# klausondrag/FOSVOS

Measured on AMD Instinct MI355X. Metric: online fine-tune frames/sec (854x480), higher is better.
Workload: dtype bf16; 1 GPU; OSVOS_VGG train_online one-shot fine-tune: 1x3x480x854 frame per step, fwd + class-balanced BCE + bwd, fused SGD step every 5 steps (BASELINE.json configs[1]); batch=1, avg_grad_every_n=5, activations=bf16 NHWC, fp32 accumulate, fp32 master weights, parallelism=single GPU

## Files before the change

fosvos_amd/csrc/common.hpp:

```cpp
#pragma once
#include <hip/hip_runtime.h>
#include <stdarg.h>
#include <algorithm>
#include <stdint.h>
#include <stdio.h>
#include <stdlib.h>
#include <string.h>

#include "../../include/fosvos_hip.h"

namespace fosvos {

extern thread_local char g_err[512];

inline int fail(int code, const char *fmt, ...) __attribute__((format(printf, 2, 3)));
inline int fail(int code, const char *fmt, ...) {
    va_list ap;
    va_start(ap, fmt);
    vsnprintf(g_err, sizeof(g_err), fmt, ap);
    va_end(ap);
    return code;
}

#define FOSVOS_HIP_CHECK(expr)                                                                         \
// ... 19 lines not shown
    } while (0)
#define FOSVOS_LAUNCH_CHECK()                            \
    do {                                                 \
        if (::fosvos::g_prof_on) ::fosvos::prof_end();   \
        FOSVOS_HIP_CHECK(hipGetLastError());             \
    } while (0)

struct WgradReduceEntry {
    const float *slabs;
    float *dw, *db;
    const float *bias_part;
    int64_t E_real, E_pad;
    int S, S_bias, Co, Cor, accumulate;
    int block_begin, n_blocks;
    int fold_begin, fold_blocks;
};
constexpr int kWgradReduceMax = 20;
struct WgradReduceTable {
    int n;
    WgradReduceEntry e[kWgradReduceMax];
};
int wgrad_impl(const uint16_t *x, const uint16_t *dy, float *dw, float *db, int N, int H, int W, int Ci, int Co,
               int accumulate, void *workspace, size_t workspace_bytes, int device, void *stream,
               WgradReduceTable *reduce, bool alone = false);
int first_wgrad_impl(const float *frame, const uint16_t *dy, float *dw, float *db, int N, int H, int W, int Co,
                     int accumulate, void *workspace, size_t workspace_bytes, int device, void *stream,
                     WgradReduceTable *reduce);
int wgrad_reduce_all(WgradReduceTable *reduce, int device, void *stream);
int wgrad_queue_reduce(const float *slabs, const float *bias_part, float *dw, float *db, int S, int S_bias, int64_t E_real,
                       int64_t E_pad, int Co, int Cor, int accumulate, WgradReduceTable *reduce, int device, void *stream);
struct HeadBwdArgs {
    const float *const *side;
    const int *hs, *ws;
    const float *const *filt, *const *filt1;
    const float *dsn_w, *fuse_w, *d_fused;
    const float *const *d_side_out;
    uint16_t *const *d_side;
    float *d_fuse_w, *d_fuse_b, *d_dsn_w, *d_dsn_b;
    int N, H, W, accumulate;
    void *workspace;
    size_t workspace_bytes;
    int device;
    int filt_uniform;
};
int head_bwd_check(const HeadBwdArgs &a);
int head_bwd_scale(const HeadBwdArgs &a, int s, void *stream);
int head_bwd_finish(const HeadBwdArgs &a, void *stream);
// ... 179 lines not shown
```

fosvos_amd/csrc/conv_wgrad.hip:

```cpp
#include <stdlib.h>

#include "common.hpp"

using namespace fosvos;

namespace {
constexpr int TH = 8;
constexpr int TPIX = TH * 16;
constexpr int HALO_W = 18;
constexpr int BCI = 64;

struct WgArgs {
    const uint16_t *x;
    const uint16_t *dy;
    float *slabs;
    float *bias_part;
    int N, H, W, Ci, Cy, Cor;
    int tiles_x, tiles_y, n_tiles, tiles_per_split;
    int lab;
    int S, n_ci, n_co, xcd_order;
};

typedef __attribute__((address_space(3))) s16x4 *lds_s16x4_ptr;

// ... 16 lines not shown
    static constexpr int NXIT = (X_PIECES + NW - 1) / NW;
    static constexpr int N_IT = 2 + NXIT;
    static_assert(Y_PIECES == 2 * NW, "two dy pieces per wave, four tile rows apart");
};

typedef __attribute__((address_space(3))) void lds_void;

__device__ __forceinline__ bf16x8 tr_pair16(const char *p, int second) {
    const s16x4 lo = __builtin_amdgcn_ds_read_tr16_b64_v4i16((lds_s16x4_ptr)(p));
    const s16x4 hi = __builtin_amdgcn_ds_read_tr16_b64_v4i16((lds_s16x4_ptr)(p + second));
    typedef __attribute__((ext_vector_type(8))) short s16x8;
    const s16x8 v = __builtin_shufflevector(lo, hi, 0, 1, 2, 3, 4, 5, 6, 7);
    return __builtin_bit_cast(bf16x8, v);
}

#pragma clang diagnostic push
#pragma clang diagnostic ignored "-Winline-asm"
__device__ __forceinline__ void dma16(const __amdgpu_buffer_rsrc_t rsrc, unsigned lds_dst, unsigned voff, unsigned soff) {
    asm volatile("s_mov_b32 m0, %0\n\ts_nop 0\n\tbuffer_load_dwordx4 %1, %2, %3 offen lds"
                 :: "s"(lds_dst), "v"(voff), "s"(rsrc), "s"(soff) : "memory", "m0");
}
#pragma clang diagnostic pop

template <bool SIDE>
__global__ __launch_bounds__(Cfg2<SIDE>::NT) __attribute__((amdgpu_waves_per_eu(SIDE ? 2 : 3, SIDE ? 4 : 3))) void k_wgrad3x3_v2(const WgArgs a) {
    using C = Cfg2<SIDE>;
    constexpr int NW = C::NW, NU = C::NU, YPX = C::YPX, Y_BYTES = C::Y_BYTES, BUF_BYTES = C::BUF_BYTES, N_IT = C::N_IT;
    extern __shared__ __attribute__((aligned(16))) char smem_w[];
    const int tid = threadIdx.x, lane = tid & 63;
    const int wave = __builtin_amdgcn_readfirstlane(tid >> 6);
    const int wc = SIDE ? 0 : wave >> 2, wi = wave & 3;
    int bid = blockIdx.x;
    if (a.xcd_order) {
        const int n_wg = gridDim.x, q8 = n_wg >> 3, r8 = n_wg & 7, xcd = bid & 7;
        bid = (xcd < r8 ? xcd * (q8 + 1) : r8 * (q8 + 1) + (xcd - r8) * q8) + (bid >> 3);
    }
    const int co_blk = bid % a.n_co, ci_blk = (bid / a.n_co) % a.n_ci, split = bid / (a.n_co * a.n_ci);
    const int ci0 = ci_blk * 64, co0 = co_blk * C::BCO;
    const int H = a.H, W = a.W;
    const unsigned lds0 = __builtin_amdgcn_readfirstlane((unsigned)(size_t)(lds_void *)smem_w);

    f32x4 acc[9][NU];
#pragma unroll
    for (int t = 0; t < 9; ++t)
#pragma unroll
        for (int u = 0; u < NU; ++u) acc[t][u] = f32x4{0.f, 0.f, 0.f, 0.f};
    float bsum[NU];
#pragma unroll
    for (int u = 0; u < NU; ++u) bsum[u] = 0.f;

    const int g = lane >> 4, q = (lane & 15) >> 2, p = lane & 3;
    const int pxl = 4 * (g & 1) + q;
    auto swz128 = [](int px, int c) { return (c ^ (2 * ((px >> 1) & 3))) * 16; };
    auto swz64 = [](int px, int c) { return (c ^ (2 * ((px >> 2) & 1))) * 16; };
    int rd_y[NU], rd_x[3];
#pragma unroll
    for (int u = 0; u < NU; ++u)
        rd_y[u] = ((4 * (g >> 1)) * 16 + pxl) * YPX + (SIDE ? swz64(pxl, p >> 1) : swz128(pxl, 2 * (2 * wc + u) + (p >> 1))) + (p & 1) * 8;
#pragma unroll
    for (int kx = 0; kx < 3; ++kx)
        rd_x[kx] = Y_BYTES + ((4 * (g >> 1)) * XROW + pxl + kx) * 128 + swz128(pxl + kx, 2 * wi + (p >> 1)) + (p & 1) * 8;
// ... 53 lines not shown
        if (++lt_y == a.tiles_y) { lt_y = 0; ++lt_n; }                                                          \
    }
#define FOSVOS_W2_PIECE_ANY(it_, img_)                                                                          \
    if constexpr ((it_) < 2) { FOSVOS_W2_PIECE_Y(it_, img_) }                                                   \
    else if constexpr ((it_) < N_IT) { FOSVOS_W2_PIECE_X(it_, img_) }
#define FOSVOS_W2_STAGE(img_)                                                                                   \
    {                                                                                                           \
        FOSVOS_W2_TILE_SCALARS()                                                                                \
        FOSVOS_W2_PIECE_ANY(0, img_) FOSVOS_W2_PIECE_ANY(1, img_) FOSVOS_W2_PIECE_ANY(2, img_)                  \
        FOSVOS_W2_PIECE_ANY(3, img_) FOSVOS_W2_PIECE_ANY(4, img_) FOSVOS_W2_PIECE_ANY(5, img_)                  \
        FOSVOS_W2_PIECE_ANY(6, img_) FOSVOS_W2_PIECE_ANY(7, img_) FOSVOS_W2_PIECE_ANY(8, img_)                  \
        FOSVOS_W2_PIECE_ANY(9, img_)                                                                            \
        FOSVOS_W2_ADVANCE()                                                                                     \
    }
    static_assert(N_IT <= 10, "piece macros cover ten pieces per wave");
#define FOSVOS_W2_PIECES_OF_ROW(R, img_)                                                                        \
    if (has_next) { FOSVOS_W2_PIECE_ANY(2 * (R), img_) FOSVOS_W2_PIECE_ANY(2 * (R) + 1, img_) }

    if (t_begin < t_end) FOSVOS_W2_STAGE(lds0)
    asm volatile("s_waitcnt vmcnt(0)" ::: "memory");
    __syncthreads();

    const bool do_bias = a.bias_part != nullptr;
    typedef __attribute__((ext_vector_type(2))) __bf16 bf16x2_t;
    auto add8 = [](const bf16x8 &f, float acc_) {
        const bf16x2_t one2 = __builtin_bit_cast(bf16x2_t, 0x3f803f80u);
        acc_ = __builtin_amdgcn_fdot2_f32_bf16(__builtin_shufflevector(f, f, 0, 1), one2, acc_, false);
        acc_ = __builtin_amdgcn_fdot2_f32_bf16(__builtin_shufflevector(f, f, 2, 3), one2, acc_, false);
        acc_ = __builtin_amdgcn_fdot2_f32_bf16(__builtin_shufflevector(f, f, 4, 5), one2, acc_, false);
        acc_ = __builtin_amdgcn_fdot2_f32_bf16(__builtin_shufflevector(f, f, 6, 7), one2, acc_, false);
        return acc_;
    };

    for (int tile = t_begin; tile < t_end; ++tile) {
        const int par = (tile - t_begin) & 1;
        const char *cur = smem_w + par * BUF_BYTES;
        const bool has_next = tile + 1 < t_end;
        const unsigned nxt_ = lds0 + (par ^ 1) * BUF_BYTES;
        FOSVOS_W2_TILE_SCALARS()
        const bool my_bias = do_bias && (tile % a.n_ci) == ci_blk && ((tile / a.n_ci) & 3) == wi;

        const char *yb[NU];
#pragma unroll
        for (int u = 0; u < NU; ++u) yb[u] = cur + rd_y[u];
        const char *xb0 = cur + rd_x[0], *xb1 = cur + rd_x[1], *xb2 = cur + rd_x[2];
        bf16x8 a0[NU], a1[NU], a2[NU], b[3], bn[3];
#pragma unroll
        for (int u = 0; u < NU; ++u) a0[u] = a1[u] = a2[u] = bf16x8{};
        bn[0] = bn[1] = bn[2] = bf16x8{};
        b[0] = tr_pair16(xb0, 1024);
        b[1] = tr_pair16(xb1, 1024);
        b[2] = tr_pair16(xb2, 1024);
#define FOSVOS_W2_ROW(R)                                                                                        \
        {                                                                                                           \
            _Pragma("unroll") for (int u = 0; u < NU; ++u) { a2[u] = a1[u]; a1[u] = a0[u]; }                        \
// ... 14 lines not shown
            }                                                                                                       \
            if constexpr ((R) >= 1 && (R) <= 4) {                                                                   \
                _Pragma("unroll") for (int kx = 0; kx < 3; ++kx)                                                    \
                _Pragma("unroll") for (int u = 0; u < NU; ++u)                                                      \
                    acc[3 + kx][u] = __builtin_amdgcn_mfma_f32_16x16x32_bf16(a1[u], b[kx], acc[3 + kx][u], 0, 0, 0); \
            }                                                                                                       \
            if constexpr ((R) < 4) {                                                                                \
                _Pragma("unroll") for (int kx = 0; kx < 3; ++kx)                                                    \
                _Pragma("unroll") for (int u = 0; u < NU; ++u)                                                      \
                    acc[kx][u] = __builtin_amdgcn_mfma_f32_16x16x32_bf16(a0[u], b[kx], acc[kx][u], 0, 0, 0);        \
                if (my_bias) {                                                                                      \
                    _Pragma("unroll") for (int u = 0; u < NU; ++u) bsum[u] = add8(a0[u], bsum[u]);                  \
                }                                                                                                   \
            }                                                                                                       \
            asm volatile("" ::: "memory");                                                                          \
            b[0] = bn[0]; b[1] = bn[1]; b[2] = bn[2];                                                               \
        }
        FOSVOS_W2_ROW(0) FOSVOS_W2_ROW(1) FOSVOS_W2_ROW(2) FOSVOS_W2_ROW(3) FOSVOS_W2_ROW(4) FOSVOS_W2_ROW(5)
        if (has_next) FOSVOS_W2_ADVANCE()
        asm volatile("s_waitcnt vmcnt(0)" ::: "memory");
        __syncthreads();
    }

    if (do_bias) {
        float *sb = reinterpret_cast<float *>(smem_w);
#pragma unroll
        for (int u = 0; u < NU; ++u) sb[(wi * 4 + g) * C::BCO + wc * 32 + u * 16 + (lane & 15)] = bsum[u];
        __syncthreads();
        if (tid < C::BCO && co0 + tid < a.Cor) {
            float acc_b = 0.f;
#pragma unroll
            for (int k = 0; k < 16; ++k) acc_b += sb[k * C::BCO + tid];
            a.bias_part[((int64_t)split * a.n_ci + ci_blk) * a.Cor + co0 + tid] = acc_b;
        }
    }
    float *slab = a.slabs + (int64_t)split * a.Cor * a.Ci * 9;
    const int ci = ci0 + wi * 16 + (lane & 15);
#pragma unroll
    for (int u = 0; u < NU; ++u)
#pragma unroll
        for (int r = 0; r < 4; ++r) {
            const int co = co0 + wc * 32 + u * 16 + 4 * g + r;
            if (co >= a.Cor || (a.lab & 1)) continue;
            float *d = slab + ((int64_t)co * a.Ci + ci) * 9;
#pragma unroll
            for (int t = 0; t < 9; ++t) d[t] = acc[t][u][r];
        }
#undef FOSVOS_W2_ROW
#undef FOSVOS_W2_PIECES_OF_ROW
#undef FOSVOS_W2_PIECE_ANY
#undef FOSVOS_W2_TILE_SCALARS
#undef FOSVOS_W2_ADVANCE
#undef FOSVOS_W2_STAGE
#undef FOSVOS_W2_PIECE_X
#undef FOSVOS_W2_PIECE_Y
}
}

constexpr int kFold = 8;

__global__ __launch_bounds__(256) void k_wgrad_fold(const WgradReduceTable t) {
    int e = 0;
    while (e + 1 < t.n && (int)blockIdx.x >= t.e[e + 1].fold_begin) ++e;
    const WgradReduceEntry &q = t.e[e];
    const int local = blockIdx.x - q.fold_begin;
    if (local >= q.fold_blocks) return;
    const int per_group = q.n_blocks;
    const int grp = local / per_group;
    const int64_t i4 = (int64_t)(local - grp * per_group) * 256 + threadIdx.x;
    if (i4 * 4 >= q.E_real) return;
    float *base = const_cast<float *>(q.slabs) + (int64_t)grp * kFold * q.E_pad + i4 * 4;
    const int n = min(kFold, q.S - grp * kFold);
    float4 v[kFold];
#pragma unroll
    for (int j = 0; j < kFold; ++j) v[j] = *reinterpret_cast<const float4 *>(base + (int64_t)min(j, n - 1) * q.E_pad);
    float4 acc = v[0];
#pragma unroll
    for (int j = 1; j < kFold; ++j)
// ... 73 lines not shown
    size_t slab_bytes, bias_bytes;
};

Plan make_plan(int N, int H, int W, int Ci, int Co, bool alone = false) {
    Plan p;
    p.side = Co % 64 != 0;
    p.Cor = p.side ? Co : roundup(Co, 64);
    p.Cy = roundup(Co, 32);
    p.tiles_x = (int)cdiv(W, 16);
    p.tiles_y = (int)cdiv(H, TH);
    p.n_tiles = p.tiles_x * p.tiles_y * N;
    const int out_blocks = p.side ? Ci / 64 : (p.Cor / 64) * (Ci / 64);
    int S = (int)cdiv(alone ? std::max(256, target_blocks()) : target_blocks(), out_blocks);
    if (S > p.n_tiles) S = p.n_tiles;
    if (S < 1) S = 1;
    p.tps = (int)cdiv(p.n_tiles, S);
    p.S = (int)cdiv(p.n_tiles, p.tps);
    p.slab_bytes = (size_t)p.S * 9 * p.Cor * Ci * sizeof(float);
    p.n_ci = Ci / 64;
    p.bias_bytes = (size_t)p.S * p.n_ci * p.Cor * sizeof(float);
    return p;
}

int check_shape(int N, int H, int W, int Ci, int Co, const char *who) {
    FOSVOS_REQUIRE(N > 0 && H > 0 && W > 0 && Ci > 0 && Co > 0, FOSVOS_E_SHAPE, "%s: bad shape", who);
    FOSVOS_REQUIRE(Ci % BCI == 0, FOSVOS_E_SHAPE, "%s: Ci=%d must be a multiple of %d", who, Ci, BCI);
    FOSVOS_REQUIRE(Co % 64 == 0 || Co == 16, FOSVOS_E_SHAPE, "%s: Co=%d must be a multiple of 64, or 16 (side_prep)", who, Co);
    FOSVOS_REQUIRE(((int64_t)N * H * W + W + 1) * std::max(Ci, roundup(Co, 32)) * 2 < 0xffffffffLL, FOSVOS_E_SHAPE,
                   "%s: a tensor of %d x %d x %d x %d bf16 exceeds the 4 GB a buffer descriptor addresses", who, N, H, W,
                   std::max(Ci, roundup(Co, 32)));
    return FOSVOS_OK;
}

int finish_or_queue(const Plan &p, float *slabs, float *bias_part, float *dw, float *db, int Ci, int Co, int accumulate,
                    WgradReduceTable *reduce, int device, hipStream_t st) {
    return fosvos::wgrad_queue_reduce(slabs, bias_part, dw, db, p.S, p.S * p.n_ci, 9LL * Co * Ci, 9LL * p.Cor * Ci, Co, p.Cor,
                                      accumulate, reduce, device, st);
}
}

extern "C" size_t fosvos_conv3x3_wgrad_workspace_bytes(int N, int H, int W, int Ci, int Co) {
    if (N <= 0 || H <= 0 || W <= 0 || Ci <= 0 || Co <= 0 || Ci % BCI != 0) return 0;
    const Plan p = make_plan(N, H, W, Ci, Co), q = make_plan(N, H, W, Ci, Co, true);
    return std::max(p.slab_bytes + p.bias_bytes, q.slab_bytes + q.bias_bytes);
}

// ... 4 lines not shown
                              nullptr);
}

extern "C" int fosvos_conv3x3_wgrad_reduce(float *dw, float *db, int N, int H, int W, int Ci, int Co, int accumulate,
                                           void *workspace, size_t workspace_bytes, int device, void *stream) {
    FOSVOS_REQUIRE(dw && workspace, FOSVOS_E_ARG, "conv3x3_wgrad_reduce: null pointer");
    if (int rc = check_shape(N, H, W, Ci, Co, "conv3x3_wgrad_reduce")) return rc;
    const Plan p = make_plan(N, H, W, Ci, Co);
    FOSVOS_REQUIRE(workspace_bytes >= p.slab_bytes + p.bias_bytes, FOSVOS_E_WORKSPACE,
                   "conv3x3_wgrad_reduce: workspace %zu < %zu", workspace_bytes, p.slab_bytes + p.bias_bytes);
    FOSVOS_ENTER(device);
    float *slabs = reinterpret_cast<float *>(workspace);
    float *bias_part = reinterpret_cast<float *>(reinterpret_cast<char *>(workspace) + p.slab_bytes);
    return finish_or_queue(p, slabs, bias_part, dw, db, Ci, Co, accumulate, nullptr, device, (hipStream_t)stream);
}

extern "C" int fosvos_conv3x3_wgrad_slabs(const uint16_t *x, const uint16_t *dy, int with_bias, int N, int H, int W, int Ci,
                                          int Co, void *workspace, size_t workspace_bytes, int device, void *stream) {
    WgradReduceTable sink;
    sink.n = 0;
    float dummy = 0.f;
    return fosvos::wgrad_impl(x, dy, &dummy, with_bias ? &dummy : nullptr, N, H, W, Ci, Co, 0, workspace, workspace_bytes,
                              device, stream, &sink);
}

int fosvos::wgrad_queue_reduce(const float *slabs, const float *bias_part, float *dw, float *db, int S, int S_bias,
                               int64_t E_real,
                               int64_t E_pad, int Co, int Cor, int accumulate, WgradReduceTable *reduce, int device,
                               void *stream) {
    WgradReduceTable local;
    local.n = 0;
    WgradReduceTable *t = reduce ? reduce : &local;
    FOSVOS_REQUIRE(t->n < kWgradReduceMax, FOSVOS_E_ARG, "wgrad: reduction queue full");
    FOSVOS_REQUIRE(E_real % 4 == 0 && E_pad % 4 == 0, FOSVOS_E_SHAPE, "wgrad: slab size must be a multiple of 4 floats");
    WgradReduceEntry &q = t->e[t->n];
    q.slabs = slabs; q.dw = dw; q.db = db; q.bias_part = db ? bias_part : nullptr;
    q.S = S; q.S_bias = S_bias; q.Co = Co; q.Cor = Cor; q.accumulate = accumulate;
    q.E_real = E_real;
    q.E_pad = E_pad;
    q.n_blocks = (int)cdiv(E_real / 4, 256);
    q.block_begin = t->n ? t->e[t->n - 1].block_begin + t->e[t->n - 1].n_blocks : 0;
    q.fold_blocks = S > kFold ? (int)cdiv(S, kFold) * q.n_blocks : 0;
    q.fold_begin = t->n ? t->e[t->n - 1].fold_begin + t->e[t->n - 1].fold_blocks : 0;
    ++t->n;
    return reduce ? FOSVOS_OK : fosvos::wgrad_reduce_all(t, device, stream);
}

int fosvos::wgrad_reduce_all(WgradReduceTable *reduce, int device, void *stream) {
    FOSVOS_REQUIRE(reduce, FOSVOS_E_ARG, "wgrad_reduce_all: null table");
    if (reduce->n == 0) return FOSVOS_OK;
    FOSVOS_ENTER(device);
    const WgradReduceEntry &last = reduce->e[reduce->n - 1];
    if (last.fold_begin + last.fold_blocks > 0) {
        FOSVOS_PROF("k_wgrad_fold", stream, 0.0);
        hipLaunchKernelGGL(k_wgrad_fold, dim3((unsigned)(last.fold_begin + last.fold_blocks)), dim3(256), 0,
                           (hipStream_t)stream, *reduce);
        FOSVOS_LAUNCH_CHECK();
    }
    FOSVOS_PROF("k_wgrad_reduce", stream, 0.0);
    hipLaunchKernelGGL(k_wgrad_reduce, dim3((unsigned)(last.block_begin + last.n_blocks)), dim3(256), 0, (hipStream_t)stream,
                       *reduce);
    FOSVOS_LAUNCH_CHECK();
    reduce->n = 0;
    return FOSVOS_OK;
}

int fosvos::wgrad_impl(const uint16_t *x, const uint16_t *dy, float *dw, float *db, int N, int H, int W, int Ci, int Co,
                       int accumulate, void *workspace, size_t workspace_bytes, int device, void *stream,
                       WgradReduceTable *reduce, bool alone) {
    FOSVOS_REQUIRE(x && dy && dw && workspace, FOSVOS_E_ARG, "conv3x3_wgrad: null pointer");
    if (int rc = check_shape(N, H, W, Ci, Co, "conv3x3_wgrad")) return rc;
    const Plan p = make_plan(N, H, W, Ci, Co, alone);
    FOSVOS_REQUIRE(workspace_bytes >= p.slab_bytes + p.bias_bytes, FOSVOS_E_WORKSPACE,
                   "conv3x3_wgrad: workspace %zu < %zu", workspace_bytes, p.slab_bytes + p.bias_bytes);
    FOSVOS_ENTER(device);
    hipStream_t st = (hipStream_t)stream;
    WgArgs a;
    a.x = x; a.dy = dy; a.slabs = reinterpret_cast<float *>(workspace);
    a.bias_part = db ? reinterpret_cast<float *>(reinterpret_cast<char *>(workspace) + p.slab_bytes) : nullptr;
    a.N = N; a.H = H; a.W = W; a.Ci = Ci; a.Cy = p.Cy; a.Cor = p.Cor;
    a.tiles_x = p.tiles_x; a.tiles_y = p.tiles_y; a.n_tiles = p.n_tiles; a.tiles_per_split = p.tps;
    a.S = p.S; a.n_ci = Ci / 64; a.n_co = p.side ? 1 : p.Cor / 64;
    {
#ifdef FOSVOS_LAB_BUILD
        static const int lab = lab_env_int("FOSVOS_WGRAD_LAB", 0);
        a.lab = lab;
#else
        a.lab = 0;
#endif
        const char *e = lab_env("FOSVOS_WGRAD_XCD");
        a.xcd_order = !(e && atoi(e) == 0);
    }
    static bool once[64][2];
    const double flops = 2.0 * N * H * W * 9.0 * Ci * Co;
    const dim3 grid((unsigned)(p.S * a.n_ci * a.n_co));
    if (p.side) {
        using C2 = v2::Cfg2<true>;
        if (device >= 0 && device < 64 && !once[device][1]) {
            FOSVOS_HIP_CHECK(hipFuncSetAttribute(reinterpret_cast<const void *>(v2::k_wgrad3x3_v2<true>),
                                                 hipFuncAttributeMaxDynamicSharedMemorySize, C2::LDS_BYTES));
            once[device][1] = true;
        }
        FOSVOS_PROF("k_wgrad3x3_v2<true>", st, flops);
        hipLaunchKernelGGL(v2::k_wgrad3x3_v2<true>, grid, dim3(C2::NT), C2::LDS_BYTES, st, a);
    } else {
        using C2 = v2::Cfg2<false>;
        if (device >= 0 && device < 64 && !once[device][0]) {
            FOSVOS_HIP_CHECK(hipFuncSetAttribute(reinterpret_cast<const void *>(v2::k_wgrad3x3_v2<false>),
                                                 hipFuncAttributeMaxDynamicSharedMemorySize, C2::LDS_BYTES));
            once[device][0] = true;
        }
        FOSVOS_PROF("k_wgrad3x3_v2<false>", st, flops);
        hipLaunchKernelGGL(v2::k_wgrad3x3_v2<false>, grid, dim3(C2::NT), C2::LDS_BYTES, st, a);
    }
    FOSVOS_LAUNCH_CHECK();
    return finish_or_queue(p, a.slabs, a.bias_part, dw, db, Ci, Co, accumulate, reduce, device, st);
}
```

fosvos_amd/fosvos_hip/__init__.py:

```python
from __future__ import annotations

import ctypes
import os
import threading
from ctypes import POINTER, c_char_p, c_float, c_int, c_int64, c_size_t, c_uint, c_void_p

_HERE = os.path.dirname(os.path.abspath(__file__))
PKG_ROOT = os.path.dirname(_HERE)
LIB_PATH = os.environ.get("FOSVOS_HIP_LIB") or os.path.join(PKG_ROOT, "lib", "libfosvos_hip.so")
HEADER_PATH = os.path.join(os.path.dirname(PKG_ROOT), "include", "fosvos_hip.h")

ABI_VERSION = 34
CONV_RELU = 1
CONV_OUT_F32 = 2
VGG_COMPACT_STAGE1 = 1


class FosvosHipError(RuntimeError):
    pass


class SgdEntry(ctypes.Structure):
    _fields_ = [("param", c_void_p), ("grad", c_void_p), ("momentum_buf", c_void_p), ("numel", c_int64),
                ("lr", c_float), ("weight_decay", c_float)]
# ... 13 lines not shown

class VggGrads(ctypes.Structure):
    _fields_ = [("conv_w", _P13), ("conv_b", _P13), ("side_w", _P4), ("side_b", _P4),
                ("dsn_w", c_void_p), ("dsn_b", c_void_p), ("fuse_w", c_void_p), ("fuse_b", c_void_p),
                ("accumulate", c_int), ("defer_join", c_int), ("bucket_events", c_int), ("last_pass_of_cycle", c_int)]

_Z4 = c_size_t * 4
_Z13 = c_size_t * 13


class VggArenaLayout(ctypes.Structure):
    _fields_ = [("total", c_size_t), ("stage_h", c_int * 5), ("stage_w", c_int * 5),
                ("act", _Z13), ("gact", _Z13), ("act_bytes", _Z13),
                ("pooled", _Z4), ("gpooled", _Z4), ("pooled_bytes", _Z4),
                ("side", _Z4), ("side_bytes", _Z4), ("dside", _Z4), ("dside_bytes", _Z4),
                ("bits0", c_size_t), ("bits0_bytes", c_size_t),
                ("ws", c_size_t), ("ws_bytes", c_size_t), ("hws", c_size_t), ("hws_bytes", c_size_t),
                ("wsa_conv", _Z13), ("wsa_conv_bytes", _Z13), ("wsa_side", _Z4), ("wsa_side_bytes", _Z4)]


class Conv3x3PlanInfo(ctypes.Structure):
    _fields_ = [("tile_h", c_int), ("tile_w", c_int), ("tile_co", c_int), ("k_splits", c_int), ("workgroups", c_int),
                ("persistent", c_int)]


class Conv2dPlanInfo(ctypes.Structure):
    _fields_ = [("cob", c_int), ("threads", c_int), ("slices", c_int), ("workgroups", c_int), ("mfma_frag_blocks", c_int),
                ("mfma_workgroups", c_int)]


class ProfileRecord(ctypes.Structure):
    _fields_ = [("name", ctypes.c_char * 96), ("launches", c_int), ("ms", ctypes.c_double), ("flops", ctypes.c_double)]


class PackEntry(ctypes.Structure):
    _fields_ = [("w", c_void_p), ("w_fwd", c_void_p), ("w_dgrad", c_void_p), ("Co", c_int), ("Ci", c_int)]



class Conv2dDesc(ctypes.Structure):
    _fields_ = [("w_packed", c_void_p), ("bias", c_void_p), ("Ci", c_int), ("Co", c_int), ("k", c_int), ("stride", c_int),
                ("kind", c_int)]


class ResnetBlock(ctypes.Structure):
    _fields_ = [("conv", Conv2dDesc * 3), ("n_convs", c_int), ("has_down", c_int), ("down", Conv2dDesc)]
# ... 26 lines not shown
    "fosvos_conv3x3_first_fwd": (c_int, [c_void_p, c_void_p, c_void_p, c_void_p, c_void_p, c_int, c_int, c_int, c_int, c_int,
                                         c_void_p]),
    "fosvos_conv3x3_dgrad_bits": (c_int, [c_void_p, c_void_p, c_void_p, c_void_p, c_void_p, c_int, c_int, c_int, c_int,
                                          c_int, c_void_p, c_size_t, c_int, c_void_p]),
    "fosvos_conv3x3_dgrad_unpool": (c_int, [c_void_p, c_void_p, c_void_p, c_void_p, c_void_p, c_int, c_int, c_int, c_int,
                                            c_int, c_void_p, c_size_t, c_int, c_void_p]),
    "fosvos_conv3x3_first_wgrad": (c_int, [c_void_p, c_void_p, c_void_p, c_void_p, c_int, c_int, c_int, c_int,
                                           c_void_p, c_size_t, c_int, c_void_p]),
    "fosvos_conv3x3_first_wgrad_workspace_bytes": (c_size_t, [c_int, c_int, c_int, c_int]),
    "fosvos_conv3x3_fwd": (c_int, [c_void_p, c_void_p, c_void_p, c_void_p, c_int, c_int, c_int, c_int, c_int, c_uint,
                                   c_void_p, c_size_t, c_int, c_void_p]),
    "fosvos_conv3x3_fwd_pool": (c_int, [c_void_p, c_void_p, c_void_p, c_void_p, c_void_p, c_int, c_int, c_int, c_int,
                                        c_int, c_uint, c_void_p, c_size_t, c_int, c_void_p]),
    "fosvos_conv3x3_workspace_bytes": (c_size_t, [c_int, c_int, c_int, c_int, c_int]),
    "fosvos_conv3x3_dgrad": (c_int, [c_void_p, c_void_p, c_void_p, c_void_p, c_void_p, c_int, c_int, c_int, c_int,
                                     c_int, c_void_p, c_size_t, c_int, c_void_p]),
    "fosvos_conv3x3_wgrad": (c_int, [c_void_p, c_void_p, c_void_p, c_void_p, c_int, c_int, c_int, c_int, c_int, c_int,
                                     c_void_p, c_size_t, c_int, c_void_p]),
    "fosvos_conv3x3_wgrad_slabs": (c_int, [c_void_p, c_void_p, c_int, c_int, c_int, c_int, c_int, c_int, c_void_p, c_size_t,
                                           c_int, c_void_p]),
    "fosvos_conv3x3_wgrad_reduce": (c_int, [c_void_p, c_void_p, c_int, c_int, c_int, c_int, c_int, c_int, c_void_p,
                                            c_size_t, c_int, c_void_p]),
    "fosvos_conv3x3_wgrad_workspace_bytes": (c_size_t, [c_int, c_int, c_int, c_int, c_int]),
    "fosvos_maxpool2x2_ceil_fwd": (c_int, [c_void_p, c_void_p, c_int, c_int, c_int, c_int, c_int, c_void_p]),
    "fosvos_maxpool2x2_ceil_bwd": (c_int, [c_void_p, c_void_p, c_void_p, c_int, c_int, c_int, c_int, c_int, c_int,
                                           c_void_p]),
    "fosvos_head_fwd": (c_int, [POINTER(c_void_p), POINTER(c_int), POINTER(c_int), POINTER(c_void_p),
                                POINTER(c_void_p), c_void_p, c_void_p, c_void_p, c_void_p, c_void_p,
                                POINTER(c_void_p), c_int, c_int, c_int, c_int, c_int, c_void_p]),
    "fosvos_head_bwd": (c_int, [POINTER(c_void_p), POINTER(c_int), POINTER(c_int), POINTER(c_void_p),
                                POINTER(c_void_p), c_void_p, c_void_p, c_void_p, POINTER(c_void_p),
                                POINTER(c_void_p), c_void_p, c_void_p, c_void_p, c_void_p, c_int, c_int, c_int, c_int,
                                c_void_p, c_size_t, c_int, c_void_p]),
    "fosvos_head_bwd_workspace_bytes": (c_size_t, [c_int, c_int, c_int]),
    "fosvos_cbce_loss": (c_int, [c_void_p, c_void_p, c_int64, c_int, c_float, c_void_p, c_void_p, c_void_p, c_size_t,
                                 c_int, c_void_p]),
    "fosvos_cbce_workspace_bytes": (c_size_t, [c_int64]),
    "fosvos_cbce_loss_frames": (c_int, [c_void_p, c_void_p, c_int64, c_int, c_int, c_float, c_void_p, c_void_p, c_void_p,
                                        c_size_t, c_int, c_void_p]),
    "fosvos_cbce_loss_frames_parts": (c_int, [c_void_p, c_void_p, c_int64, c_int, c_int, c_float, c_void_p, c_void_p,
                                              c_void_p, c_size_t, c_int, c_int, c_void_p]),
    "fosvos_cbce_multi_workspace_bytes": (c_size_t, [c_int64, c_int, c_int]),
    "fosvos_cbce_loss_frames_multi": (c_int, [POINTER(c_void_p), c_void_p, c_int64, c_int, c_int, c_int, POINTER(c_float),
                                              c_void_p, POINTER(c_void_p), c_void_p, c_size_t, c_int, c_int, c_void_p]),
    "fosvos_cbce_loss_batch_counts": (c_int, [c_void_p, c_void_p, c_int64, c_int, c_float, c_void_p, c_void_p, c_void_p,
                                              c_void_p, c_size_t, c_int, c_void_p]),
# ... 194 lines not shown
```

fosvos_amd/fosvos_hip/ops.py:

```python
from __future__ import annotations

import ctypes
import math
from typing import List, Optional, Sequence, Tuple

import torch

from . import CONV_OUT_F32, CONV_RELU, check, int_array4, lib, limits, ptr_array4

_BF16 = torch.bfloat16
_F32 = torch.float32


def _need(t: torch.Tensor, dtype, what: str, dtype_error=TypeError) -> torch.Tensor:
    if not t.is_cuda:
        raise RuntimeError(f"{what}: tensor must live on the GPU (the HIP path has no CPU fallback)")
    if t.dtype != dtype:
        raise dtype_error(f"{what}: expected {dtype}, got {t.dtype}")
    if not t.is_contiguous():
        raise ValueError(f"{what}: tensor must be contiguous")
    return t


def _ctx(t: torch.Tensor) -> Tuple[int, int]:
# ... 339 lines not shown

def conv3x3_wgrad(x: torch.Tensor, dy: torch.Tensor, ci: int, co: int, with_bias: bool = True,
                  dw: Optional[torch.Tensor] = None, db: Optional[torch.Tensor] = None, accumulate: bool = False):
    _need(x, _BF16, "conv3x3_wgrad x"); _need(dy, _BF16, "conv3x3_wgrad dy")
    n, h, wd, cx = x.shape
    if cx != ci or tuple(dy.shape) != (n, h, wd, _ru(co, 32)):
        raise ValueError(f"conv3x3_wgrad: shapes x={tuple(x.shape)} dy={tuple(dy.shape)} do not match Ci={ci} Co={co}")
    L = lib()
    if dw is None:
        if accumulate:
            raise ValueError("conv3x3_wgrad: accumulate needs an existing dw")
        dw = torch.empty((co, ci, 3, 3), dtype=_F32, device=x.device)
    if with_bias and db is None:
        if accumulate:
            raise ValueError("conv3x3_wgrad: accumulate needs an existing db")
        db = torch.empty((co,), dtype=_F32, device=x.device)
    _need(dw, _F32, "conv3x3_wgrad dw")
    ws, wsn = _WS.get(L.fosvos_conv3x3_wgrad_workspace_bytes(n, h, wd, ci, co), x.device)
    _launch("conv3x3_wgrad_slabs", x, x.data_ptr(), dy.data_ptr(), 1 if with_bias else 0, n, h, wd, ci, co, ws, wsn,
            record="conv3x3_wgrad", flops=2.0 * n * h * wd * 9 * ci * co, nbytes=n * h * wd * 2 * (ci + dy.shape[3]))
    _launch("conv3x3_wgrad_reduce", x, dw.data_ptr(), _p(db) if with_bias else None, n, h, wd, ci, co, 1 if accumulate else 0,
            ws, wsn, record="wgrad_reduce", nbytes=4 * 9 * ci * co * 3)
    return dw, (db if with_bias else None)


def conv3x3_wgrad_one_call(x: torch.Tensor, dy: torch.Tensor, ci: int, co: int, with_bias: bool = True):
    _need(x, _BF16, "conv3x3_wgrad x"); _need(dy, _BF16, "conv3x3_wgrad dy")
    n, h, wd, _ = x.shape
    L = lib()
    dw = torch.empty((co, ci, 3, 3), dtype=_F32, device=x.device)
    db = torch.empty((co,), dtype=_F32, device=x.device) if with_bias else None
    ws, wsn = _WS.get(L.fosvos_conv3x3_wgrad_workspace_bytes(n, h, wd, ci, co), x.device)
    _launch("conv3x3_wgrad", x, x.data_ptr(), dy.data_ptr(), dw.data_ptr(), _p(db), n, h, wd, ci, co, 0, ws, wsn, record=False)
    return dw, db


def maxpool_fwd(x: torch.Tensor) -> torch.Tensor:
    _need(x, _BF16, "maxpool_fwd")
    n, h, w, c = x.shape
    y = torch.empty((n, (h + 1) // 2, (w + 1) // 2, c), dtype=_BF16, device=x.device)
    _launch("maxpool2x2_ceil_fwd", x, x.data_ptr(), y.data_ptr(), n, h, w, c, record="maxpool_fwd", nbytes=2 * (x.numel() + y.numel()))
    return y


def maxpool_bwd(x: torch.Tensor, dy: torch.Tensor, relu_mask: bool = True) -> torch.Tensor:
    _need(x, _BF16, "maxpool_bwd x"); _need(dy, _BF16, "maxpool_bwd dy")
# ... 1211 lines not shown
```

include/fosvos_hip.h:

```cpp
#ifndef FOSVOS_HIP_H
#define FOSVOS_HIP_H

#include <stddef.h>
#include <stdint.h>

#ifdef __cplusplus
extern "C" {
#endif

#define FOSVOS_ABI_VERSION 34

#define FOSVOS_OK 0
#define FOSVOS_E_SHAPE (-1)
#define FOSVOS_E_ARG (-2)
#define FOSVOS_E_WORKSPACE (-3)
#define FOSVOS_E_HIP (-4)

#define FOSVOS_CONV_RELU 1u
#define FOSVOS_CONV_OUT_F32 2u
#define FOSVOS_CONV_FP32_MATH 4u

int fosvos_abi_version(void);

typedef struct fosvos_profile_record {
// ... 71 lines not shown
    int k_splits;
    int workgroups;
    int persistent;
} fosvos_conv3x3_plan_info;
int fosvos_conv3x3_plan(int N, int H, int W, int in_ch, int out_ch, fosvos_conv3x3_plan_info *out);
int fosvos_conv3x3_fwd_plan(int N, int H, int W, int in_ch, int out_ch, unsigned flags, fosvos_conv3x3_plan_info *out);
int fosvos_conv3x3_dgrad(const uint16_t *dy, const uint16_t *w_dgrad_packed, const uint16_t *relu_src,
                         const uint16_t *addend, uint16_t *dx, int N, int H, int W, int Ci, int Co, void *workspace,
                         size_t workspace_bytes, int device, void *stream);
int fosvos_conv3x3_dgrad_bits(const uint16_t *dy, const uint16_t *w_dgrad_packed, const uint8_t *relu_bits,
                              const uint16_t *addend, uint16_t *dx, int N, int H, int W, int Ci, int Co, void *workspace,
                              size_t workspace_bytes, int device, void *stream);
int fosvos_conv3x3_dgrad_unpool(const uint16_t *dy, const uint16_t *w_dgrad_packed, const uint16_t *x,
                                const uint16_t *d_pooled, uint16_t *dx, int N, int H, int W, int Ci, int Co,
                                void *workspace, size_t workspace_bytes, int device, void *stream);
int fosvos_conv3x3_wgrad(const uint16_t *x, const uint16_t *dy, float *dw_oihw, float *dbias, int N, int H, int W,
                         int Ci, int Co, int accumulate, void *workspace, size_t workspace_bytes, int device,
                         void *stream);
size_t fosvos_conv3x3_wgrad_workspace_bytes(int N, int H, int W, int Ci, int Co);
int fosvos_conv3x3_wgrad_slabs(const uint16_t *x, const uint16_t *dy, int with_bias, int N, int H, int W, int Ci, int Co,
                               void *workspace, size_t workspace_bytes, int device, void *stream);
int fosvos_conv3x3_wgrad_reduce(float *dw_oihw, float *dbias, int N, int H, int W, int Ci, int Co, int accumulate,
                                void *workspace, size_t workspace_bytes, int device, void *stream);

int fosvos_maxpool2x2_ceil_fwd(const uint16_t *x, uint16_t *y, int N, int H, int W, int C, int device, void *stream);
int fosvos_maxpool2x2_ceil_bwd(const uint16_t *x, const uint16_t *dy, uint16_t *dx, int N, int H, int W, int C,
                               int relu_mask, int device, void *stream);
int fosvos_maxpool2x2_ceil_bwd_codes(const uint32_t *codes, const uint16_t *dy, uint16_t *dx, int N, int H, int W, int C,
                                     int device, void *stream);

int fosvos_head_fwd(const float *const side[4], const int hs[4], const int ws[4], const float *const filt[4],
                    const float *const filt1[4], const float *dsn_w , const float *dsn_b ,
                    const float *fuse_w , const float *fuse_b , float *fused,
                    float *const side_out[4] , int N, int H, int W, int filt_uniform, int device,
                    void *stream);
int fosvos_head_bwd(const float *const side[4], const int hs[4], const int ws[4], const float *const filt[4],
                    const float *const filt1[4], const float *dsn_w, const float *fuse_w, const float *d_fused,
                    const float *const d_side_out[4], uint16_t *const d_side[4], float *d_fuse_w, float *d_fuse_b,
                    float *d_dsn_w, float *d_dsn_b, int N, int H, int W, int filt_uniform ,
                    void *workspace, size_t workspace_bytes, int device, void *stream);
size_t fosvos_head_bwd_workspace_bytes(int N, int H, int W);

int fosvos_cbce_loss(const float *logits, const float *label, int64_t numel, int size_average, float grad_scale,
                     float *loss_out, float *grad, void *workspace, size_t workspace_bytes, int device,
                     void *stream);
size_t fosvos_cbce_workspace_bytes(int64_t numel);
// ... 240 lines not shown
```

Baseline: 1267 frames/s.

## Add warp-specialized ring-buffered wgrad kernel for Co≥512 conv layers

Adds a new 3x3 weight-gradient kernel in which four producer waves stream dy and x tiles into a three-deep LDS ring via buffer-to-LDS DMA, while eight MFMA waves consume them. The goal is to overlap global loads with matrix math instead of having the same waves alternate between staging and compute. By default it is selected only for layers with more than 256 output channels, with an env mask to choose others, and the epilogue is factored into a shared helper. The cost is a larger LDS footprint and more threads per workgroup, which can lower occupancy, plus hand-tuned vmcnt waits that depend on piece counts.

```diff
diff --git a/fosvos_amd/csrc/common.hpp b/fosvos_amd/csrc/common.hpp
--- a/fosvos_amd/csrc/common.hpp
+++ b/fosvos_amd/csrc/common.hpp
@@ -65,7 +65,7 @@
 };
 int wgrad_impl(const uint16_t *x, const uint16_t *dy, float *dw, float *db, int N, int H, int W, int Ci, int Co,
                int accumulate, void *workspace, size_t workspace_bytes, int device, void *stream,
-               WgradReduceTable *reduce, bool alone = false);
+               WgradReduceTable *reduce, bool alone = false, int form = -1);
 int first_wgrad_impl(const float *frame, const uint16_t *dy, float *dw, float *db, int N, int H, int W, int Co,
                      int accumulate, void *workspace, size_t workspace_bytes, int device, void *stream,
                      WgradReduceTable *reduce);
diff --git a/fosvos_amd/csrc/conv_wgrad.hip b/fosvos_amd/csrc/conv_wgrad.hip
--- a/fosvos_amd/csrc/conv_wgrad.hip
+++ b/fosvos_amd/csrc/conv_wgrad.hip
@@ -62,6 +62,63 @@
 }
 #pragma clang diagnostic pop
 
+struct WgId {
+    int co_blk, ci_blk, split;
+};
+__device__ __forceinline__ WgId wg_id(const WgArgs &a) {
+    int bid = blockIdx.x;
+    if (a.xcd_order) {
+        const int n_wg = gridDim.x, q8 = n_wg >> 3, r8 = n_wg & 7, xcd = bid & 7;
+        bid = (xcd < r8 ? xcd * (q8 + 1) : r8 * (q8 + 1) + (xcd - r8) * q8) + (bid >> 3);
+    }
+    return {bid % a.n_co, (bid / a.n_co) % a.n_ci, bid / (a.n_co * a.n_ci)};
+}
+
+template <bool SIDE, int NU>
+__device__ __forceinline__ void store_partials(const WgArgs &a, char *smem, const f32x4 (&acc)[9][NU], const float (&bsum)[NU],
+                                               const WgId &id, int wc, int wi, bool mfma_wave) {
+    constexpr int BCO = SIDE ? 16 : 64;
+    const int tid = threadIdx.x, lane = tid & 63, g = lane >> 4;
+    const int ci0 = id.ci_blk * 64, co0 = id.co_blk * BCO;
+    if (a.bias_part != nullptr) {
+        float *sb = reinterpret_cast<float *>(smem);
+        if (mfma_wave) {
+#pragma unroll
+            for (int u = 0; u < NU; ++u) sb[(wi * 4 + g) * BCO + wc * 32 + u * 16 + (lane & 15)] = bsum[u];
+        }
+        __syncthreads();
+        if (tid < BCO && co0 + tid < a.Cor) {
+            float acc_b = 0.f;
+#pragma unroll
+            for (int k = 0; k < 16; ++k) acc_b += sb[k * BCO + tid];
+            a.bias_part[((int64_t)id.split * a.n_ci + id.ci_blk) * a.Cor + co0 + tid] = acc_b;
+        }
+    }
+    if (!mfma_wave) return;
+    float *slab = a.slabs + (int64_t)id.split * a.Cor * a.Ci * 9;
+    const int ci = ci0 + wi * 16 + (lane & 15);
+#pragma unroll
+    for (int u = 0; u < NU; ++u)
+#pragma unroll
+        for (int r = 0; r < 4; ++r) {
+            const int co = co0 + wc * 32 + u * 16 + 4 * g + r;
+            if (co >= a.Cor || (a.lab & 1)) continue;
+            float *d = slab + ((int64_t)co * a.Ci + ci) * 9;
+#pragma unroll
+            for (int t = 0; t < 9; ++t) d[t] = acc[t][u][r];
+        }
+}
+
+__device__ __forceinline__ float add8(const bf16x8 &f, float acc_) {
+    typedef __attribute__((ext_vector_type(2))) __bf16 bf16x2_t;
+    const bf16x2_t one2 = __builtin_bit_cast(bf16x2_t, 0x3f803f80u);
+    acc_ = __builtin_amdgcn_fdot2_f32_bf16(__builtin_shufflevector(f, f, 0, 1), one2, acc_, false);
+    acc_ = __builtin_amdgcn_fdot2_f32_bf16(__builtin_shufflevector(f, f, 2, 3), one2, acc_, false);
+    acc_ = __builtin_amdgcn_fdot2_f32_bf16(__builtin_shufflevector(f, f, 4, 5), one2, acc_, false);
+    acc_ = __builtin_amdgcn_fdot2_f32_bf16(__builtin_shufflevector(f, f, 6, 7), one2, acc_, false);
+    return acc_;
+}
+
 template <bool SIDE>
 __global__ __launch_bounds__(Cfg2<SIDE>::NT) __attribute__((amdgpu_waves_per_eu(SIDE ? 2 : 3, SIDE ? 4 : 3))) void k_wgrad3x3_v2(const WgArgs a) {
     using C = Cfg2<SIDE>;
@@ -70,13 +127,9 @@
     const int tid = threadIdx.x, lane = tid & 63;
     const int wave = __builtin_amdgcn_readfirstlane(tid >> 6);
     const int wc = SIDE ? 0 : wave >> 2, wi = wave & 3;
-    int bid = blockIdx.x;
-    if (a.xcd_order) {
-        const int n_wg = gridDim.x, q8 = n_wg >> 3, r8 = n_wg & 7, xcd = bid & 7;
-        bid = (xcd < r8 ? xcd * (q8 + 1) : r8 * (q8 + 1) + (xcd - r8) * q8) + (bid >> 3);
-    }
-    const int co_blk = bid % a.n_co, ci_blk = (bid / a.n_co) % a.n_ci, split = bid / (a.n_co * a.n_ci);
-    const int ci0 = ci_blk * 64, co0 = co_blk * C::BCO;
+    const WgId id = wg_id(a);
+    const int ci_blk = id.ci_blk, split = id.split;
+    const int ci0 = ci_blk * 64, co0 = id.co_blk * C::BCO;
     const int H = a.H, W = a.W;
     const unsigned lds0 = __builtin_amdgcn_readfirstlane((unsigned)(size_t)(lds_void *)smem_w);
 
@@ -176,15 +229,6 @@
     __syncthreads();
 
     const bool do_bias = a.bias_part != nullptr;
-    typedef __attribute__((ext_vector_type(2))) __bf16 bf16x2_t;
-    auto add8 = [](const bf16x8 &f, float acc_) {
-        const bf16x2_t one2 = __builtin_bit_cast(bf16x2_t, 0x3f803f80u);
-        acc_ = __builtin_amdgcn_fdot2_f32_bf16(__builtin_shufflevector(f, f, 0, 1), one2, acc_, false);
-        acc_ = __builtin_amdgcn_fdot2_f32_bf16(__builtin_shufflevector(f, f, 2, 3), one2, acc_, false);
-        acc_ = __builtin_amdgcn_fdot2_f32_bf16(__builtin_shufflevector(f, f, 4, 5), one2, acc_, false);
-        acc_ = __builtin_amdgcn_fdot2_f32_bf16(__builtin_shufflevector(f, f, 6, 7), one2, acc_, false);
-        return acc_;
-    };
 
     for (int tile = t_begin; tile < t_end; ++tile) {
         const int par = (tile - t_begin) & 1;
@@ -245,31 +289,7 @@
         __syncthreads();
     }
 
-    if (do_bias) {
-        float *sb = reinterpret_cast<float *>(smem_w);
-#pragma unroll
-        for (int u = 0; u < NU; ++u) sb[(wi * 4 + g) * C::BCO + wc * 32 + u * 16 + (lane & 15)] = bsum[u];
-        __syncthreads();
-        if (tid < C::BCO && co0 + tid < a.Cor) {
-            float acc_b = 0.f;
-#pragma unroll
-            for (int k = 0; k < 16; ++k) acc_b += sb[k * C::BCO + tid];
-            a.bias_part[((int64_t)split * a.n_ci + ci_blk) * a.Cor + co0 + tid] = acc_b;
-        }
-    }
-    float *slab = a.slabs + (int64_t)split * a.Cor * a.Ci * 9;
-    const int ci = ci0 + wi * 16 + (lane & 15);
-#pragma unroll
-    for (int u = 0; u < NU; ++u)
-#pragma unroll
-        for (int r = 0; r < 4; ++r) {
-            const int co = co0 + wc * 32 + u * 16 + 4 * g + r;
-            if (co >= a.Cor || (a.lab & 1)) continue;
-            float *d = slab + ((int64_t)co * a.Ci + ci) * 9;
-#pragma unroll
-            for (int t = 0; t < 9; ++t) d[t] = acc[t][u][r];
-        }
-#undef FOSVOS_W2_ROW
+    store_partials<SIDE, NU>(a, smem_w, acc, bsum, id, wc, wi, true);
 #undef FOSVOS_W2_PIECES_OF_ROW
 #undef FOSVOS_W2_PIECE_ANY
 #undef FOSVOS_W2_TILE_SCALARS
@@ -277,6 +297,134 @@
 #undef FOSVOS_W2_STAGE
 #undef FOSVOS_W2_PIECE_X
 #undef FOSVOS_W2_PIECE_Y
+}
+}
+
+namespace ring {
+using namespace v2;
+using C = Cfg2<false>;
+constexpr int NMW = 8, NPW = 4;
+constexpr int NT = 64 * (NMW + NPW);
+constexpr int DEPTH = 3;
+constexpr int LDS_BYTES = DEPTH * C::BUF_BYTES;
+constexpr int PIECES = C::BUF_BYTES / 1024;
+constexpr int PIECES_PER_WAVE = (PIECES + NPW - 1) / NPW;
+static_assert(NPW * 4 == C::Y_PIECES, "the first four rounds of pieces are dy's, the others x's");
+static_assert(PIECES % NPW == 2 && PIECES_PER_WAVE == 12, "vmcnt immediates below");
+
+__global__ __launch_bounds__(NT) __attribute__((amdgpu_waves_per_eu(3, 3))) void k_wgrad3x3_ring(const WgArgs a) {
+    constexpr int NU = C::NU, YPX = C::YPX, Y_BYTES = C::Y_BYTES, BUF_BYTES = C::BUF_BYTES, XROW = v2::XROW;
+    extern __shared__ __attribute__((aligned(16))) char smem_w[];
+    const int tid = threadIdx.x, lane = tid & 63;
+    const int wave = __builtin_amdgcn_readfirstlane(tid >> 6);
+    const bool producer = wave >= NMW;
+    const int wc = (wave >> 2) & 1, wi = wave & 3;
+    const WgId id = wg_id(a);
+    const int ci_blk = id.ci_blk;
+    const int ci0 = ci_blk * 64, co0 = id.co_blk * C::BCO;
+    const int H = a.H, W = a.W;
+    const unsigned lds0 = __builtin_amdgcn_readfirstlane((unsigned)(size_t)(v2::lds_void *)smem_w);
+
+    f32x4 acc[9][NU];
+#pragma unroll
+    for (int t = 0; t < 9; ++t)
+#pragma unroll
+        for (int u = 0; u < NU; ++u) acc[t][u] = f32x4{0.f, 0.f, 0.f, 0.f};
+    float bsum[NU];
+#pragma unroll
+    for (int u = 0; u < NU; ++u) bsum[u] = 0.f;
+
+    const int g = lane >> 4, q = (lane & 15) >> 2, p = lane & 3;
+    const int pxl = 4 * (g & 1) + q;
+    auto swz128 = [](int px, int c) { return (c ^ (2 * ((px >> 1) & 3))) * 16; };
+    int rd_y[NU], rd_x[3];
+#pragma unroll
+    for (int u = 0; u < NU; ++u) rd_y[u] = ((4 * (g >> 1)) * 16 + pxl) * YPX + swz128(pxl, 2 * (2 * wc + u) + (p >> 1)) + (p & 1) * 8;
+#pragma unroll
+    for (int kx = 0; kx < 3; ++kx)
+        rd_x[kx] = Y_BYTES + ((4 * (g >> 1)) * XROW + pxl + kx) * 128 + swz128(pxl + kx, 2 * wi + (p >> 1)) + (p & 1) * 8;
+
+    const int t_begin = id.split * a.tiles_per_split;
+    const int n_my = max(min(t_begin + a.tiles_per_split, a.n_tiles) - t_begin, 0);
+
+    const int pw = wave - NMW;
+    const int ppx = lane >> 3, slot = lane & 7;
+    const int64_t halo_shift = (int64_t)(W + 1) * a.Ci;
+    const unsigned y_total = (unsigned)((int64_t)a.N * H * W * a.Cy * 2), x_total = (unsigned)(((int64_t)a.N * H * W * a.Ci + halo_shift) * 2);
+    const auto y_rsrc = __builtin_amdgcn_make_buffer_rsrc(const_cast<uint16_t *>(a.dy), 0, y_total, 0x00020000);
+    const auto x_rsrc = __builtin_amdgcn_make_buffer_rsrc(const_cast<uint16_t *>(a.x) - halo_shift, 0, x_total, 0x00020000);
+    int lt_x = t_begin % a.tiles_x, lt_y = (t_begin / a.tiles_x) % a.tiles_y, lt_n = t_begin / (a.tiles_x * a.tiles_y);
+    auto stage_tile = [&](unsigned img) {
+        const int y0 = lt_y * TH, x0 = lt_x * 16;
+        const int vrows = H - y0, vcols = W - x0;
+        const int64_t org = ((int64_t)lt_n * H + y0) * W + x0;
+        const unsigned ysoff = (unsigned)(org * a.Cy * 2), xsoff = (unsigned)(org * a.Ci * 2);
+#pragma unroll
+        for (int k = 0; k < PIECES_PER_WAVE; ++k) {
+            const int pc = pw + NPW * k;
+            if (k < 4) {
+                const int pix = pc * 8 + ppx, ty = pix >> 4, tx = pix & 15;
+                const bool in = ty < vrows && tx < vcols;
+                const unsigned v = in ? (unsigned)(((ty * W + tx) * a.Cy + co0 + (slot ^ (2 * ((tx >> 1) & 3))) * 8) * 2) : ~0u;
+                v2::dma16(y_rsrc, img + pc * 1024, v, ysoff);
+            } else if (pc < PIECES) {
+                const int xp = pc - C::Y_PIECES, pix = xp * 8 + ppx, hy = pix / XROW, hx = pix - hy * XROW;
+                const bool in = hx < HALO_W && hy >= 1 - y0 && hy <= vrows && hx >= 1 - x0 && hx <= vcols;
+                const unsigned v = in ? (unsigned)(((hy * W + hx) * a.Ci + ci0 + (slot ^ (2 * ((hx >> 1) & 3))) * 8) * 2) : ~0u;
+                v2::dma16(x_rsrc, img + Y_BYTES + xp * 1024, v, xsoff);
+            }
+        }
+        if (++lt_x == a.tiles_x) {
+            lt_x = 0;
+            if (++lt_y == a.tiles_y) { lt_y = 0; ++lt_n; }
+        }
+    };
+    auto wait_older = [&](bool newer) {
+        if (!newer) asm volatile("s_waitcnt vmcnt(0)" ::: "memory");
+        else if (pw < PIECES % NPW) asm volatile("s_waitcnt vmcnt(12)" ::: "memory");
+        else asm volatile("s_waitcnt vmcnt(11)" ::: "memory");
+    };
+
+    if (producer) {
+        if (n_my > 0) stage_tile(lds0);
+        if (n_my > 1) stage_tile(lds0 + BUF_BYTES);
+        wait_older(n_my > 1);
+    }
+    __syncthreads();
+
+    const bool do_bias = a.bias_part != nullptr;
+#define FOSVOS_W2_PIECES_OF_ROW(R, img_)
+    int cur_slot = 0, fill_slot = 2;
+    for (int i = 0; i < n_my; ++i) {
+        if (producer) {
+            const bool more = i + 2 < n_my;
+            if (more) stage_tile(lds0 + fill_slot * BUF_BYTES);
+            wait_older(more);
+        } else {
+            const int tile = t_begin + i;
+            const char *cur = smem_w + cur_slot * BUF_BYTES;
+            const bool my_bias = do_bias && (tile % a.n_ci) == ci_blk && ((tile / a.n_ci) & 3) == wi;
+            const char *yb[NU];
+#pragma unroll
+            for (int u = 0; u < NU; ++u) yb[u] = cur + rd_y[u];
+            const char *xb0 = cur + rd_x[0], *xb1 = cur + rd_x[1], *xb2 = cur + rd_x[2];
+            bf16x8 a0[NU], a1[NU], a2[NU], b[3], bn[3];
+#pragma unroll
+            for (int u = 0; u < NU; ++u) a0[u] = a1[u] = a2[u] = bf16x8{};
+            bn[0] = bn[1] = bn[2] = bf16x8{};
+            b[0] = tr_pair16(xb0, 1024);
+            b[1] = tr_pair16(xb1, 1024);
+            b[2] = tr_pair16(xb2, 1024);
+            FOSVOS_W2_ROW(0) FOSVOS_W2_ROW(1) FOSVOS_W2_ROW(2) FOSVOS_W2_ROW(3) FOSVOS_W2_ROW(4) FOSVOS_W2_ROW(5)
+            asm volatile("s_waitcnt lgkmcnt(0)" ::: "memory");
+        }
+        __syncthreads();
+        cur_slot = cur_slot == DEPTH - 1 ? 0 : cur_slot + 1;
+        fill_slot = fill_slot == DEPTH - 1 ? 0 : fill_slot + 1;
+    }
+#undef FOSVOS_W2_PIECES_OF_ROW
+#undef FOSVOS_W2_ROW
+    store_partials<false, NU>(a, smem_w, acc, bsum, id, wc, wi, !producer);
 }
 }
 
@@ -396,6 +544,15 @@
     return p;
 }
 
+constexpr int kRingAlone = 1, kRingCo64 = 2, kRingCo128 = 4, kRingCo256 = 8, kRingCo512 = 16;
+constexpr int kRingDefault = kRingCo512;
+int wgrad_form(const Plan &p, int Co, bool alone) {
+    if (p.side) return FOSVOS_WGRAD_V2;
+    const int mask = lab_env_int("FOSVOS_WGRAD_FORM", kRingDefault);
+    const int cls = alone ? kRingAlone : Co <= 64 ? kRingCo64 : Co <= 128 ? kRingCo128 : Co <= 256 ? kRingCo256 : kRingCo512;
+    return (mask & cls) ? FOSVOS_WGRAD_RING : FOSVOS_WGRAD_V2;
+}
+
 int check_shape(int N, int H, int W, int Ci, int Co, const char *who) {
     FOSVOS_REQUIRE(N > 0 && H > 0 && W > 0 && Ci > 0 && Co > 0, FOSVOS_E_SHAPE, "%s: bad shape", who);
     FOSVOS_REQUIRE(Ci % BCI == 0, FOSVOS_E_SHAPE, "%s: Ci=%d must be a multiple of %d", who, Ci, BCI);
@@ -446,6 +603,28 @@
     float dummy = 0.f;
     return fosvos::wgrad_impl(x, dy, &dummy, with_bias ? &dummy : nullptr, N, H, W, Ci, Co, 0, workspace, workspace_bytes,
                               device, stream, &sink);
+}
+
+extern "C" int fosvos_conv3x3_wgrad_slabs_as(int form, const uint16_t *x, const uint16_t *dy, int with_bias, int N, int H, int W,
+                                             int Ci, int Co, void *workspace, size_t workspace_bytes, int device, void *stream) {
+    FOSVOS_REQUIRE(form == FOSVOS_WGRAD_V2 || form == FOSVOS_WGRAD_RING, FOSVOS_E_ARG, "conv3x3_wgrad_slabs_as: unknown form %d", form);
+    FOSVOS_REQUIRE(form == FOSVOS_WGRAD_V2 || Co % 64 == 0, FOSVOS_E_SHAPE, "conv3x3_wgrad_slabs_as: side_prep (Co=%d) has the v2 form only", Co);
+    WgradReduceTable sink;
+    sink.n = 0;
+    float dummy = 0.f;
+    return fosvos::wgrad_impl(x, dy, &dummy, with_bias ? &dummy : nullptr, N, H, W, Ci, Co, 0, workspace, workspace_bytes,
+                              device, stream, &sink, false, form);
+}
+
+extern "C" int fosvos_conv3x3_wgrad_plan(int N, int H, int W, int Ci, int Co, fosvos_conv3x3_wgrad_plan_info *out) {
+    FOSVOS_REQUIRE(out, FOSVOS_E_ARG, "conv3x3_wgrad_plan: null output");
+    if (int rc = check_shape(N, H, W, Ci, Co, "conv3x3_wgrad_plan")) return rc;
+    const Plan p = make_plan(N, H, W, Ci, Co);
+    out->form = wgrad_form(p, Co, false);
+    out->tiles = p.n_tiles; out->tiles_per_split = p.tps; out->splits = p.S;
+    out->workgroups = p.S * p.n_ci * (p.side ? 1 : p.Cor / 64);
+    out->slab_rows = p.Cor;
+    return FOSVOS_OK;
 }
 
 int fosvos::wgrad_queue_reduce(const float *slabs, const float *bias_part, float *dw, float *db, int S, int S_bias,
@@ -491,10 +670,11 @@
 
 int fosvos::wgrad_impl(const uint16_t *x, const uint16_t *dy, float *dw, float *db, int N, int H, int W, int Ci, int Co,
                        int accumulate, void *workspace, size_t workspace_bytes, int device, void *stream,
-                       WgradReduceTable *reduce, bool alone) {
+                       WgradReduceTable *reduce, bool alone, int form) {
     FOSVOS_REQUIRE(x && dy && dw && workspace, FOSVOS_E_ARG, "conv3x3_wgrad: null pointer");
     if (int rc = check_shape(N, H, W, Ci, Co, "conv3x3_wgrad")) return rc;
     const Plan p = make_plan(N, H, W, Ci, Co, alone);
+    if (form < 0) form = wgrad_form(p, Co, alone);
     FOSVOS_REQUIRE(workspace_bytes >= p.slab_bytes + p.bias_bytes, FOSVOS_E_WORKSPACE,
                    "conv3x3_wgrad: workspace %zu < %zu", workspace_bytes, p.slab_bytes + p.bias_bytes);
     FOSVOS_ENTER(device);
@@ -515,7 +695,7 @@
         const char *e = lab_env("FOSVOS_WGRAD_XCD");
         a.xcd_order = !(e && atoi(e) == 0);
     }
-    static bool once[64][2];
+    static bool once[64][3];
     const double flops = 2.0 * N * H * W * 9.0 * Ci * Co;
     const dim3 grid((unsigned)(p.S * a.n_ci * a.n_co));
     if (p.side) {
@@ -527,6 +707,14 @@
         }
         FOSVOS_PROF("k_wgrad3x3_v2<true>", st, flops);
         hipLaunchKernelGGL(v2::k_wgrad3x3_v2<true>, grid, dim3(C2::NT), C2::LDS_BYTES, st, a);
+    } else if (form == FOSVOS_WGRAD_RING) {
+        if (device >= 0 && device < 64 && !once[device][2]) {
+            FOSVOS_HIP_CHECK(hipFuncSetAttribute(reinterpret_cast<const void *>(ring::k_wgrad3x3_ring),
+                                                 hipFuncAttributeMaxDynamicSharedMemorySize, ring::LDS_BYTES));
+            once[device][2] = true;
+        }
+        FOSVOS_PROF("k_wgrad3x3_ring", st, flops);
+        hipLaunchKernelGGL(ring::k_wgrad3x3_ring, grid, dim3(ring::NT), ring::LDS_BYTES, st, a);
     } else {
         using C2 = v2::Cfg2<false>;
         if (device >= 0 && device < 64 && !once[device][0]) {
diff --git a/fosvos_amd/fosvos_hip/__init__.py b/fosvos_amd/fosvos_hip/__init__.py
--- a/fosvos_amd/fosvos_hip/__init__.py
+++ b/fosvos_amd/fosvos_hip/__init__.py
@@ -59,6 +59,11 @@
 class Conv3x3PlanInfo(ctypes.Structure):
     _fields_ = [("tile_h", c_int), ("tile_w", c_int), ("tile_co", c_int), ("k_splits", c_int), ("workgroups", c_int),
                 ("persistent", c_int)]
+
+
+class WgradPlanInfo(ctypes.Structure):
+    _fields_ = [("form", c_int), ("tiles", c_int), ("tiles_per_split", c_int), ("splits", c_int), ("workgroups", c_int),
+                ("slab_rows", c_int)]
 
 
 class Conv2dPlanInfo(ctypes.Structure):
@@ -131,6 +136,9 @@
     "fosvos_conv3x3_wgrad_reduce": (c_int, [c_void_p, c_void_p, c_int, c_int, c_int, c_int, c_int, c_int, c_void_p,
                                             c_size_t, c_int, c_void_p]),
     "fosvos_conv3x3_wgrad_workspace_bytes": (c_size_t, [c_int, c_int, c_int, c_int, c_int]),
+    "fosvos_conv3x3_wgrad_plan": (c_int, [c_int, c_int, c_int, c_int, c_int, POINTER(WgradPlanInfo)]),
+    "fosvos_conv3x3_wgrad_slabs_as": (c_int, [c_int, c_void_p, c_void_p, c_int, c_int, c_int, c_int, c_int, c_int, c_void_p,
+                                              c_size_t, c_int, c_void_p]),
     "fosvos_maxpool2x2_ceil_fwd": (c_int, [c_void_p, c_void_p, c_int, c_int, c_int, c_int, c_int, c_void_p]),
     "fosvos_maxpool2x2_ceil_bwd": (c_int, [c_void_p, c_void_p, c_void_p, c_int, c_int, c_int, c_int, c_int, c_int,
                                            c_void_p]),
diff --git a/fosvos_amd/fosvos_hip/ops.py b/fosvos_amd/fosvos_hip/ops.py
--- a/fosvos_amd/fosvos_hip/ops.py
+++ b/fosvos_amd/fosvos_hip/ops.py
@@ -385,6 +385,16 @@
     _launch("conv3x3_wgrad_reduce", x, dw.data_ptr(), _p(db) if with_bias else None, n, h, wd, ci, co, 1 if accumulate else 0,
             ws, wsn, record="wgrad_reduce", nbytes=4 * 9 * ci * co * 3)
     return dw, (db if with_bias else None)
+
+
+WGRAD_V2, WGRAD_RING = 0, 1
+
+
+def conv3x3_wgrad_plan(n: int, h: int, w: int, ci: int, co: int) -> dict:
+    from . import WgradPlanInfo
+    info = WgradPlanInfo()
+    check(lib().fosvos_conv3x3_wgrad_plan(n, h, w, ci, co, ctypes.byref(info)), "conv3x3_wgrad_plan")
+    return {k: getattr(info, k) for k, _ in WgradPlanInfo._fields_}
 
 
 def conv3x3_wgrad_one_call(x: torch.Tensor, dy: torch.Tensor, ci: int, co: int, with_bias: bool = True):
diff --git a/include/fosvos_hip.h b/include/fosvos_hip.h
--- a/include/fosvos_hip.h
+++ b/include/fosvos_hip.h
@@ -117,6 +117,19 @@
                                void *workspace, size_t workspace_bytes, int device, void *stream);
 int fosvos_conv3x3_wgrad_reduce(float *dw_oihw, float *dbias, int N, int H, int W, int Ci, int Co, int accumulate,
                                 void *workspace, size_t workspace_bytes, int device, void *stream);
+#define FOSVOS_WGRAD_V2 0
+#define FOSVOS_WGRAD_RING 1
+typedef struct fosvos_conv3x3_wgrad_plan_info {
+    int form;
+    int tiles;
+    int tiles_per_split;
+    int splits;
+    int workgroups;
+    int slab_rows;
+} fosvos_conv3x3_wgrad_plan_info;
+int fosvos_conv3x3_wgrad_plan(int N, int H, int W, int Ci, int Co, fosvos_conv3x3_wgrad_plan_info *out);
+int fosvos_conv3x3_wgrad_slabs_as(int form, const uint16_t *x, const uint16_t *dy, int with_bias, int N, int H, int W, int Ci,
+                                  int Co, void *workspace, size_t workspace_bytes, int device, void *stream);
 
 int fosvos_maxpool2x2_ceil_fwd(const uint16_t *x, uint16_t *y, int N, int H, int W, int C, int device, void *stream);
 int fosvos_maxpool2x2_ceil_bwd(const uint16_t *x, const uint16_t *dy, uint16_t *dx, int N, int H, int W, int C,
```

After: 1266 frames/s. Within noise of the previous version (-0.1%).
